# jamornsriwasansak/evplp

Hardware: AMD Instinct MI355X
Metric: Mpaths/s (higher is better)
Workload: dtype f32

## Files before the change

### evplp_amd/csrc/kernels.h

```cpp
#pragma once
#include "evplp_types.h"

namespace evplp {

struct PrimaryArgs {
    SceneDev sc; StripDev st; CamBasis cam;
    float jitter[2]; int32_t clear_light; int32_t pad;
    float4 *g_pos, *g_nrm, *g_dif, *g_phg, *g_light;
    float4 *tile_box;
    const char *cuts; int32_t cut_gw_log2, cut_gh_log2, cut_groups_x, pad2;
};
struct PrimaryCutArgs {
    const BvhNode *nodes; StripDev st; CamBasis cam;
    int32_t tiles_x, tiles_y, gw_log2, gh_log2, groups_x, groups_y;
    char *cuts;
};
void launch_primary_cuts(const PrimaryCutArgs &a, hipStream_t s);
#ifndef EVPLP_PRIMARY_BLOCKS
#define EVPLP_PRIMARY_BLOCKS 1
#endif
#ifndef EVPLP_PRIMARY_BLOCK_LOG2
#define EVPLP_PRIMARY_BLOCK_LOG2 2
#endif

struct LightTraceArgs {
    SceneDev sc;
    uint32_t rng_seed, path_begin, path_count, photons_per_path;
    evplp_record *records;
    int32_t *stack_overflow;
    uint32_t overflow_stride, pad;
};
#ifndef EVPLP_LT_STACK
#define EVPLP_LT_STACK 20
#endif
constexpr int kLtLdsStack = EVPLP_LT_STACK;
inline int lt_overflow_entries(const SceneDev &sc) {
    const int generic = 3 * ((sc.bvh_depth + 1) / 2) + 4;
    const int worst = sc.stack4_entries > 0 && sc.stack4_entries < generic ? sc.stack4_entries : generic;
    return worst > kLtLdsStack ? worst - kLtLdsStack : 0;
}

struct PassCounters {
    unsigned long long rays;
    unsigned long long nodes;
    unsigned long long pairs;
    unsigned long long aux;
    unsigned long long hist[64];
    unsigned long long shard_rays[64], shard_shaded[64];
    unsigned long long nonfinite;
};
#ifndef EVPLP_DEBUG_NAN
#define EVPLP_DEBUG_NAN 0
#endif
constexpr int kCounterShards = 64;

struct GatherArgs {
    SceneDev sc; StripDev st;
    const float4 *g_pos, *g_nrm, *g_dif, *g_phg;
    const evplp_record *vpls;
    const uint32_t *vpl_src_index;
    const uint32_t *nvpl;
    evplp_frame_params fp;
    float pdf_mc2; int32_t pad0;
    float4 *out;
    float4 *partial;
    size_t partial_stride;
    PassCounters *counters;
    int32_t splits_per_wave;
    int32_t block_h_log2;
    int32_t group_first, group_count;
    unsigned long long *vsl_masks; int32_t masks_per_split; int32_t pad1;
    const char *cuts; uint32_t cut_vpl_stride; int32_t cut_gw_log2, cut_gh_log2, cut_groups_x;
    int32_t band_first, band_rows, cut_group_row_first;
    int32_t item_deal;
    unsigned long long *block_cost;
};
struct AdaptArgs { const int4 *tiles; const float4 *snap; int32_t n1, pad; };
constexpr int kCutEntries = 8;
constexpr int kCutNodes = kCutEntries / 2;
constexpr int kCutSlotBytes = kCutNodes * 64;
struct CutArgs {
    const BvhNode *nodes;
    const float4 *tile_box;
    int32_t tiles_x, tiles_y;
    int32_t gw_log2, gh_log2;
    int32_t groups_x, groups_y;
    int32_t group_row_first, pad;
    const evplp_record *vpls; const uint32_t *nvpl; uint32_t vpl_stride;
    char *cuts;
    const int4 *adapt_tiles;
};
void launch_gather_cuts(const CutArgs &a, hipStream_t s);
void launch_tile_boxes(const StripDev &st, const float4 *g_pos, float4 *tile_box, int tiles_x, int tiles_y, hipStream_t s);
#ifndef EVPLP_VPL_SPLIT
#define EVPLP_VPL_SPLIT 128
#endif
constexpr int kVplSplit = EVPLP_VPL_SPLIT;
#ifndef EVPLP_GATHER_K
#define EVPLP_GATHER_K 2
#endif
constexpr int kDefaultSplitsPerWave = EVPLP_GATHER_K;

struct PathTraceArgs {
    SceneDev sc; StripDev st;
    const float4 *g_pos, *g_nrm, *g_dif, *g_phg;
    float camera_pos[3]; uint32_t rng_seed;
    uint32_t max_bounces, do_accumulate;
    float4 *out;
    PassCounters *counters;
};

constexpr int kPtBatchMaxSamples = 64;
constexpr int kPtBatchMaxTiles = 1 << 25;
constexpr size_t kPtBatchSlotBytes = 4 * 64 * sizeof(float4);
struct PtBatchSamples { float jitter[kPtBatchMaxSamples][2]; uint32_t seed[kPtBatchMaxSamples]; };
__host__ __device__ inline int32_t pt_tile_samples(int32_t mode, int4 r, int32_t S) {
    return mode == 0 ? S : mode == 1 ? (r.x == 0 ? S : 0) : (r.w < 0 || r.w > S ? S : r.w);
}
__host__ __device__ inline bool gather_tile_takes(int4 r, int32_t phase, int32_t S) {
    return r.w < 0 || phase < (r.w < S ? r.w : S);
}
constexpr int kGatherBudgetMaxWindow = 64;
void launch_gather_budget_mask(const int4 *tiles, int32_t ntiles, int32_t phase, int32_t window, int4 *mask, hipStream_t s);
void launch_gather_budget_step(int4 *tiles, const int4 *mask, int32_t ntiles, hipStream_t s);
void launch_gather_reduce_budget(const GatherArgs &a, int stencil_test, const int4 *tiles, const int4 *mask, float4 *snap, int32_t n1, hipStream_t s);
struct PtBatchChunk {
    const uint32_t *table; const int32_t *total;
    int32_t item_first, item_count;
    float4 *staging;
    unsigned long long cut_mask;
};
void launch_pt_batch_table(const int4 *tiles, int32_t ntiles, int32_t mode, int32_t samples, int32_t *first, uint32_t *table, hipStream_t s);
void launch_pt_batch_primary(const PrimaryArgs &a, const PtBatchSamples &sm, const PtBatchChunk &ch, hipStream_t s);
void launch_pt_batch_trace(const PathTraceArgs &a, const PtBatchSamples &sm, const PtBatchChunk &ch, hipStream_t s);
void launch_pt_batch_accumulate(const StripDev &st, float4 *plane, const int32_t *first, int32_t ntiles, const PtBatchChunk &ch, hipStream_t s);
void launch_pt_batch_close(const StripDev &st, int4 *tiles, int32_t mode, const int32_t *first, const float4 *snap, float4 *out, int32_t n_after, int32_t ntiles, hipStream_t s);

constexpr int kSummaryShards = 1024, kSummaryStride = 32, kSummaryFinal = kSummaryShards * kSummaryStride;
constexpr int kSummaryHeavy = kSummaryFinal + 8;
#ifndef EVPLP_BIN_CHUNKS
#define EVPLP_BIN_CHUNKS 1
#endif
constexpr int kBinChunks = EVPLP_BIN_CHUNKS;
constexpr int kBinGroup = 256 * kBinChunks;
constexpr int kSegCap = 4 * kBinGroup;
#ifndef EVPLP_SCATTER_G
#define EVPLP_SCATTER_G 2
#endif
constexpr int kScatterG = EVPLP_SCATTER_G;
constexpr int kMaxBuckets = 1024;
constexpr int kBucketTilesLog2 = 7;
constexpr int kMaxBucketTilesLog2 = 9;
struct SplatArgs {
    StripDev st; CamBasis cam;
    evplp_frame_params fp;
    const float4 *g_pos, *g_nrm, *g_dif, *g_phg;
    const evplp_record *records; uint32_t num_records;
    float4 *out;
    uint32_t *tile_pairs;
    float4 *tile_box;
    uint32_t *tile_cursor;
    uint32_t *bin_items;
    uint32_t bin_stride;
    uint32_t *seg;
    uint16_t *seg_off;
    uint32_t *big_list;
    uint32_t *big_count;
    int32_t num_bin_groups, bucket_w_log2, bucket_h_log2, buckets_x, num_buckets;
    uint32_t *bin_items_tmp;
    float4 *compact;
    uint32_t *overflow;
    uint32_t *summary;
    int32_t tiles_x, tiles_y; int32_t deterministic; int32_t boxes_valid;
    PassCounters *counters;
    const float4 *proxy_slabs; const float *proxy_hm; int32_t proxy_count; float proxy_rin, proxy_rout;
    uint32_t *tile_frags;
    uint32_t *heavy_list; uint8_t *tile_flags; uint32_t heavy_cap, heavy_threshold;
};
constexpr int kMaxProxySlabs = EVPLP_MAX_PROXY_PLANES;
constexpr float kProxyOpen = 1.0e15f;
constexpr int kSplatTile = 8;
constexpr int kCompactF4 = 4;

inline size_t lane_stack_bytes(const SceneDev &sc) { return (size_t)(sc.bvh_depth + 2) * 64 * sizeof(int32_t); }
inline size_t lane_stack_bytes4(const SceneDev &sc) {
    const int generic = 3 * ((sc.bvh_depth + 1) / 2) + 4;
    const int entries = sc.stack4_entries > 0 ? (sc.stack4_entries < generic ? sc.stack4_entries : generic) : generic;
    return (size_t)entries * 64 * sizeof(int32_t);
}

void launch_primary(const PrimaryArgs &a, hipStream_t s);
void launch_light_trace(const LightTraceArgs &a, hipStream_t s);
void launch_compact_vpl(const evplp_record *records, uint32_t nrec, evplp_record *out, uint32_t *src_index,
                        uint32_t *count_out, hipStream_t s);
void launch_gather_vpl_items(const GatherArgs &a, hipStream_t s, const AdaptArgs &ad = AdaptArgs{});
void launch_gather_vsl(const GatherArgs &a, hipStream_t s, const AdaptArgs &ad = AdaptArgs{});
int gather_launch_tiles(const GatherArgs &a);
void launch_gather_reduce(const GatherArgs &a, int stencil_test, hipStream_t s, const AdaptArgs &ad = AdaptArgs{});
void launch_gather_lvc(const GatherArgs &a, const evplp_record *records, hipStream_t s);
void launch_path_trace(const PathTraceArgs &a, hipStream_t s, const AdaptArgs &ad = AdaptArgs{});
void launch_splat_bin(const SplatArgs &a, hipStream_t s);
void launch_splat_tiles(const SplatArgs &a, bool split_tiles, hipStream_t s, hipEvent_t dominant_begin, hipEvent_t dominant_end);
void launch_resolve(const StripDev &st, const float4 *vpl, const float4 *pm, const float4 *light,
                    float vs, float ps, float ls, int mask_emitter, int gamma, float *out_rgb, hipStream_t s);
void launch_assemble_strips(const StripDev &st, int nranks, const uint32_t *owner, int chunk_rows, const float *gathered, float *frame, hipStream_t s, int channels = 3);
struct ShardPlanes { const float4 *p[64]; };
void launch_reduce_shards(const ShardPlanes &src, int n, int first_nonzero, size_t count, float4 *out, int num_cus, hipStream_t s);
void launch_fill_zero(void *p, size_t bytes, hipStream_t s);
struct RowError { double num, rel, rel_kept, kept; };
static_assert(sizeof(RowError) == 32, "RowError must be 32 bytes");
void launch_frame_error(const StripDev &st, const float *rgb, const float *ref, const uint8_t *keep, RowError *rows, hipStream_t s);
struct NoisePlanes { double *q; float4 *prev, *start; size_t stride; };
struct NoiseMoments { const double *q, *s; const float4 *prev, *start; size_t stride; };
void launch_noise_pool(const NoiseMoments &src, bool first, double *q, double *s_out, size_t n, hipStream_t s);
struct AdaptTiles { const int4 *tiles; int32_t tiles_x, pad; double n, scale; };
void launch_noise_fold(const NoisePlanes &m, const float4 *vpl, const float4 *pm, const StripDev &st, const AdaptTiles &at, int32_t k, hipStream_t s);
void launch_noise_rows(const StripDev &st, const NoiseMoments &m, double K, double B, double s2K, const float4 *light, float ls, int mask_emitter,
                       const float *rgb, const uint8_t *keep, RowError *rows, const AdaptTiles &at, hipStream_t s);
void launch_noise_variance(const StripDev &st, const NoiseMoments &m, double K, double B, double s2K, float *out_rgb, const AdaptTiles &at, hipStream_t s);
void launch_adaptive_retire(const StripDev &st, const NoiseMoments &m, double K, double B, double s2K, const float4 *light, float ls, int mask_emitter,
                            const float *rgb, double tau, int4 *tiles, int32_t tiles_x, int32_t tiles_y, int32_t n, const float4 *vpl, float4 *snap, hipStream_t s);

void launch_noise_fold_budget(const NoisePlanes &m, const StripDev &st, int4 *tiles, const float4 *snap, int32_t ntiles, hipStream_t s);
void launch_tile_noise(const StripDev &st, const NoiseMoments &m, double K, double B, double s2K, const float4 *light, float ls, int mask_emitter,
                       const float *rgb, const AdaptTiles &at, int32_t ntiles, double *out, hipStream_t s);

struct DenoisePixel { float4 u, pos, nrm, albedo, rgb; };
static_assert(sizeof(DenoisePixel) == 80, "DenoisePixel must be 80 bytes");
constexpr int kDenoiseFloats = (int)(sizeof(DenoisePixel) / sizeof(float));
void launch_denoise_prepare(const StripDev &st, const float *rgb, const float *var, const float4 *pos, const float4 *nrm, const float4 *dif,
                            const float4 *phg, const float4 *light, float4 *out, hipStream_t s);
struct DenoiseLevelArgs {
    const DenoisePixel *frame; const float4 *in; float4 *out;
    int32_t W, rows, in_step, h;
    float sigma_l, sigma_n, sigma_x_r, pad;
};
void launch_denoise_level(const DenoiseLevelArgs &a, hipStream_t s);
void launch_denoise_finish(const DenoisePixel *frame, const float4 *u, size_t n, float *out_rgb, hipStream_t s);

struct TemporalPrev { float4 pos, nrm; };
constexpr int kTemporalPrevFloats = (int)(sizeof(TemporalPrev) / sizeof(float));
void launch_prev_pose(const PrimaryArgs &a, const float *prev_v, TemporalPrev *prev, float4 *debug, hipStream_t s);
void launch_pose_snapshot(const TriAttr *attrs, int32_t ntri, float *prev_v, hipStream_t s);
int temporal_count_slots(int W, int rows);
struct TemporalArgs {
    DenoisePixel *frame; const TemporalPrev *prev; const float4 *h_in; float4 *h_out; uint4 *counts;
    size_t px;
    int32_t W, rows, H, has_history;
    CamBasis cam, prev_cam;
    float sigma_x_r, normal_cos, max_history, pad;
};
void launch_temporal_accumulate(const TemporalArgs &a, hipStream_t s);

}
// ... 1 lines not shown
```

### evplp_amd/csrc/kernels_gather.hip

```cpp
#include "device_common.hpp"
#include "kernels.h"
#include <algorithm>

namespace evplp {

constexpr int kRecF4 = sizeof(evplp_record) / 16;

struct Pixel {
    V3 p1, n1, rd, rs; float e; V3 wi10;
};

struct Vpl {
    V3 pos, n, flux, fdir, rd, rs; float psel, e;
};
EV_DEV Vpl load_vpl(const float4 *r) {
    Vpl v; float4 a = r[0], b = r[1], c = r[2], d = r[3], e = r[4], f = r[5];
    v.pos = v3(a); v.n = v3(b); v.psel = b.w; v.flux = v3(c); v.fdir = v3(d); v.rd = v3(e); v.rs = v3(f); v.e = f.w;
    return v;
}

EV_DEV float phong_eval_f_hw(V3 out, V3 in, V3 n, float e) {
    V3 r = reflect(-in, n);
    float d = fmaxf(dot(out, r), 0.0f);
    if (d <= 0.000001f) return 0.0f;
    return (e + 2.0f) * __builtin_amdgcn_exp2f(e * __builtin_amdgcn_logf(d)) * EV_INV_PI * 0.5f;
}

template <bool PXL = false>
EV_DEV V3 vpl_shade(const evplp_frame_params &fp, float pdf_mc2, const Pixel &px, const Vpl &v, V3 v12, float c1c2, const float *wi10_lds = nullptr, bool px_glossy = true) {
    float dist2 = dot(v12, v12);
    V3 wi12 = v12 * __builtin_amdgcn_rsqf(dist2);
    float ph2 = 0.0f;
    if (v.rs.x != 0.0f || v.rs.y != 0.0f || v.rs.z != 0.0f) {
        if (v.e == 0.0f) { V3 r = reflect(-v.fdir, v.n); ph2 = fmaxf(dot(-wi12, r), 0.0f) <= 0.000001f ? 0.0f : (v.e + 2.0f) * 1.0f * EV_INV_PI * 0.5f; }
        else ph2 = phong_eval_f_hw(-wi12, v.fdir, v.n, v.e);
    }
    float ph1 = 0.0f;
    V3 prs = PXL ? v3(0.f, 0.f, 0.f) : px.rs;
    if (PXL ? px_glossy : ballot64(px.rs.x != 0.0f || px.rs.y != 0.0f || px.rs.z != 0.0f) != 0ull) {
        ph1 = phong_eval_f_hw(wi10_lds ? v3(wi10_lds[0], wi10_lds[64], wi10_lds[128]) : px.wi10, wi12, px.n1, PXL ? wi10_lds[576] : px.e);
        if (PXL) prs = v3(wi10_lds[384], wi10_lds[448], wi10_lds[512]);
    }
    const V3 prd = PXL ? v3(wi10_lds[192], wi10_lds[256], wi10_lds[320]) : px.rd;
    V3 brdf2 = v.rd * EV_INV_PI + v.rs * ph2;
    V3 brdf1 = prd * EV_INV_PI + prs * ph1;
    float g21 = c1c2 * __builtin_amdgcn_rcpf(dist2 * dist2);
    const uint32_t mode = fp.mis_mode;
    if (mode == 0u) return v.flux * brdf1 * brdf2 * g21;
    if (mode <= 3u) {
        float pdf_de = g21 * EV_INV_PI * v.psel;
        if (!(v.rs.x <= 0.000001f))
            pdf_de += ph2 * ((v.e + 1.0f) * __builtin_amdgcn_rcpf(v.e + 2.0f)) * fmaxf(dot(px.n1, wi12), 0.0f) * __builtin_amdgcn_rcpf(dist2) * (1.0f - v.psel);
        float w;
        if (mode == 1u) w = fp.pdf_mc * __builtin_amdgcn_rcpf(fp.pdf_mc + pdf_de);
        else if (mode == 2u) w = fp.pdf_mc > pdf_de ? 1.0f : 0.0f;
        else { float a2 = pdf_mc2, b2 = pdf_de * pdf_de; w = a2 * __builtin_amdgcn_rcpf(a2 + b2); }
        return (v.flux * w) * brdf1 * brdf2 * g21;
    }
    if (mode == 4u) return (v.flux * fminf(g21, fp.clamping_value)) * brdf1 * brdf2;
    V3 x = (brdf1 * g21) * brdf2;
    x = v3(fminf(x.x, fp.clamping_value), fminf(x.y, fp.clamping_value), fminf(x.z, fp.clamping_value));
    return v.flux * x;
}

struct Item { int x, ly, gy, group; bool in_image, has_tile; uint32_t p; };
#ifndef EVPLP_GROUP_ORDER
#define EVPLP_GROUP_ORDER 0
#endif
#ifndef EVPLP_XCD_TIMES
#define EVPLP_XCD_TIMES 0
#endif
#ifndef EVPLP_XCD_ROTATE
#define EVPLP_XCD_ROTATE 2
#endif
struct ItemIx { int tx, ty, sg, tile_l, blk; };
template <bool RANGE = false>
EV_DEV ItemIx item_index(const GatherArgs &a, int b) {
    const int tiles_x = (a.st.W + 7) >> 3;
    const int groups = RANGE ? a.group_count : kVplSplit / a.splits_per_wave;
    const bool grp = EVPLP_GROUP_ORDER == 1 && a.cuts != nullptr;
    const int gwl = grp ? a.cut_gw_log2 : 0, ghl = grp ? a.cut_gh_log2 : 0, gl = gwl + ghl;
    const int xcd = b & 7, j = b >> 3;
    const int q = j & ((1 << gl) - 1);
    const int r = a.item_deal ? b : j >> gl;
    const int unit_j = r / groups;
    const int unit = a.item_deal ? unit_j : unit_j * 8 + xcd;
    const int shl = a.block_h_log2, bwl = 3 - gwl, bhl = shl - ghl, nbx = (tiles_x + 7) >> 3;
    const int l = unit & ((1 << (bwl + bhl)) - 1);
    ItemIx ix;
    ix.blk = a.band_first * nbx + (unit >> (bwl + bhl));
    const int rot = EVPLP_XCD_ROTATE == 0 ? 0 : EVPLP_XCD_ROTATE == 1 ? (l >> bwl) + ix.blk : (l >> bwl) + (ix.blk % nbx) + ((ix.blk / nbx) << bhl);
    const int ux = ((ix.blk % nbx) << bwl) | ((l + rot) & ((1 << bwl) - 1)), uy = ((ix.blk / nbx) << bhl) | (l >> bwl);
    ix.tx = (ux << gwl) | (q & ((1 << gwl) - 1)); ix.ty = (uy << ghl) | (q >> gwl);
    ix.sg = r - unit_j * groups;
    ix.tile_l = (unit << gl) | q;
    return ix;
}
template <bool RANGE = false>
EV_DEV Item item_setup(const GatherArgs &a, int lane, int b) {
    const StripDev &st = a.st;
    const int tiles_x = (st.W + 7) >> 3, tiles_y = (st.local_rows + 7) >> 3;
    const int sh = 1 << a.block_h_log2, nbx = (tiles_x + 7) >> 3, nby = (tiles_y + sh - 1) >> a.block_h_log2;
    const ItemIx ix = item_index<RANGE>(a, b);
    Item t;
    t.group = (RANGE ? a.group_first : 0) + ix.sg;
    t.has_tile = ix.blk < nbx * (a.band_rows > 0 ? min(nby, a.band_first + a.band_rows) : nby) && ix.tx < tiles_x && ix.ty < tiles_y;
    t.x = ix.tx * 8 + (lane & 7); t.ly = ix.ty * 8 + (lane >> 3);
    const int cly = max(min(t.ly, st.local_rows - 1), 0);
    t.gy = st.global_row(cly);
    t.has_tile = t.has_tile && __builtin_amdgcn_readfirstlane(t.gy) < st.H;
    t.in_image = t.has_tile && t.x < st.W && t.ly < st.local_rows && t.gy < st.H;
    t.p = (uint32_t)cly * (uint32_t)st.W + (uint32_t)min(t.x, st.W - 1);
    return t;
}

template <bool RANGE = false>
EV_DEV uint32_t item_texel(const GatherArgs &a, int lane, int b) {
    const StripDev &st = a.st;
    const ItemIx ix = item_index<RANGE>(a, b);
    const int x = ix.tx * 8 + (lane & 7), ly = ix.ty * 8 + (lane >> 3);
    return (uint32_t)max(min(ly, st.local_rows - 1), 0) * (uint32_t)st.W + (uint32_t)min(x, st.W - 1);
}

EV_DEV uint32_t item_cut_group(const GatherArgs &a, const Item &t) {
    const int tx = __builtin_amdgcn_readfirstlane(t.x) >> 3, ty = __builtin_amdgcn_readfirstlane(t.ly) >> 3;
    return (uint32_t)(((ty >> a.cut_gh_log2) - a.cut_group_row_first) * a.cut_groups_x + (tx >> a.cut_gw_log2));
}
EV_DEV bool tile_retired(const GatherArgs &a, const AdaptArgs &ad, const Item &t) {
    const int tx = __builtin_amdgcn_readfirstlane(t.x) >> 3, ty = __builtin_amdgcn_readfirstlane(t.ly) >> 3;
    const uint32_t off = (uint32_t)(ty * ((a.st.W + 7) >> 3) + tx) * (uint32_t)sizeof(int4);
    int nt;
    asm volatile("s_load_dword %0, %1, %2\n\ts_waitcnt lgkmcnt(0)" : "=s"(nt) : "s"(ad.tiles), "s"(off) : "memory");
    return nt != 0;
}

#ifndef EVPLP_CUT_RING
#define EVPLP_CUT_RING 3
#endif
#ifndef EVPLP_PX_LDS
#define EVPLP_PX_LDS 1
#endif
constexpr int kGatherPxFloats = 64 * (EVPLP_PX_LDS ? 10 : 3);
#ifndef EVPLP_GATHER_WAVES
#define EVPLP_GATHER_WAVES 8
#endif

EV_DEV Vpl fetch_vpl(const evplp_record *r) {
    const v16i ra = *reinterpret_cast<const v16i *>(r);
    const v8i rb = *reinterpret_cast<const v8i *>(reinterpret_cast<const int *>(r) + 16);
    Vpl v;
    v.pos = v3(f_of(ra[0]), f_of(ra[1]), f_of(ra[2])); v.n = v3(f_of(ra[4]), f_of(ra[5]), f_of(ra[6])); v.psel = f_of(ra[7]);
    v.flux = v3(f_of(ra[8]), f_of(ra[9]), f_of(ra[10])); v.fdir = v3(f_of(ra[12]), f_of(ra[13]), f_of(ra[14]));
    v.rd = v3(f_of(rb[0]), f_of(rb[1]), f_of(rb[2])); v.rs = v3(f_of(rb[4]), f_of(rb[5]), f_of(rb[6])); v.e = f_of(rb[7]);
    return v;
}
EV_DEV void fetch_vpl_head(const evplp_record *vpls, uint32_t i, V3 &pos, V3 &n, float &psel) {
    const v8i ra = sload8(vpls, i * (uint32_t)sizeof(evplp_record));
    pos = v3(f_of(ra[0]), f_of(ra[1]), f_of(ra[2])); n = v3(f_of(ra[4]), f_of(ra[5]), f_of(ra[6])); psel = f_of(ra[7]);
}
EV_DEV void fetch_vpl_tail(const evplp_record *vpls, uint32_t i, Vpl &v) {
    const v16i rb = sload16(vpls, i * (uint32_t)sizeof(evplp_record) + 32u);
    v.flux = v3(f_of(rb[0]), f_of(rb[1]), f_of(rb[2])); v.fdir = v3(f_of(rb[4]), f_of(rb[5]), f_of(rb[6]));
    v.rd = v3(f_of(rb[8]), f_of(rb[9]), f_of(rb[10])); v.rs = v3(f_of(rb[12]), f_of(rb[13]), f_of(rb[14])); v.e = f_of(rb[15]);
}

#if EVPLP_GATHER_TIMES
__device__ unsigned long long g_gather_times[2 * 131072];
extern "C" int evplp_debug_gather_times(unsigned long long *out, int n) { return (int)hipMemcpyFromSymbol(out, HIP_SYMBOL(g_gather_times), sizeof(unsigned long long) * (size_t)n); }
#endif
EV_DEV void item_cost_add(const GatherArgs &a, int ty, unsigned long long t0, int waves) {
    const unsigned long long dt = __builtin_amdgcn_s_memrealtime() - t0;
    if (threadIdx.x == 0) atomicAdd(&a.block_cost[(ty * 8) / a.st.strip_rows], dt * 8ull / (unsigned long long)waves);
}
template <bool CUT, bool COST = false, bool ADAPT = false>
__attribute__((amdgpu_num_vgpr(kWalkKernelVgprs)))
__global__ __launch_bounds__(64, EVPLP_GATHER_WAVES) void gather_vpl_kernel(GatherArgs a, AdaptArgs ad) {
    unsigned long long t_cost = 0ull;
    if constexpr (COST) t_cost = __builtin_amdgcn_s_memrealtime();
#if EVPLP_GATHER_TIMES
    const unsigned long long t_start = __builtin_amdgcn_s_memrealtime();
#endif
    extern __shared__ float s_dyn[];
    float *const s_wi10 = s_dyn, *const s_lvl = s_dyn + kGatherPxFloats;
    const int lane = threadIdx.x;
    const Item t = item_setup(a, lane, (int)blockIdx.x);
    if (!t.has_tile) return;
    if constexpr (ADAPT) { if (tile_retired(a, ad, t)) return; }
    const uint32_t p = t.p;

    Pixel px;
    float4 gp = a.g_pos[p], gn = a.g_nrm[p], gd = a.g_dif[p], gs = a.g_phg[p];
    px.p1 = v3(gp); px.n1 = v3(gn); px.rd = v3(gd); px.rs = v3(gs); px.e = gs.w;
#ifndef EVPLP_WI10_LDS
#define EVPLP_WI10_LDS 1
#endif
    {
        const V3 w = normalize(v3(a.fp.camera_pos) - px.p1);
        s_wi10[lane] = w.x; s_wi10[64 + lane] = w.y; s_wi10[128 + lane] = w.z;
        px.wi10 = EVPLP_WI10_LDS ? v3(0.f, 0.f, 0.f) : w;
    }
    bool px_glossy = true;
    if constexpr (EVPLP_PX_LDS != 0) {
        static_assert(EVPLP_WI10_LDS != 0, "EVPLP_PX_LDS continues the LDS column of the view direction");
        s_wi10[192 + lane] = px.rd.x; s_wi10[256 + lane] = px.rd.y; s_wi10[320 + lane] = px.rd.z;
        s_wi10[384 + lane] = px.rs.x; s_wi10[448 + lane] = px.rs.y; s_wi10[512 + lane] = px.rs.z; s_wi10[576 + lane] = px.e;
        px_glossy = ballot64(px.rs.x != 0.0f || px.rs.y != 0.0f || px.rs.z != 0.0f) != 0ull;
        px.rd = v3(0.f, 0.f, 0.f); px.rs = v3(0.f, 0.f, 0.f); px.e = 0.0f;
    }
    const bool valid = t.in_image && gp.w != 0.0f;

    const uint32_t nvpl = *a.nvpl;
    const int k = a.splits_per_wave;
    const char *node_base = pinned(reinterpret_cast<const char *>(a.sc.nodes)), *leaf_base = pinned(reinterpret_cast<const char *>(a.sc.leaves));
    const evplp_record *vpls = pinned(a.vpls);
    const char *cuts_g = nullptr;
    if constexpr (CUT) cuts_g = pinned(a.cuts + (size_t)item_cut_group(a, t) * a.cut_vpl_stride * (size_t)kCutSlotBytes);
    V3 total = v3(0.f, 0.f, 0.f);
    uint32_t rays = t.in_image ? 0x80000000u : 0u, shaded = 0;
#if EVPLP_TRAVERSAL_STATS
    int32_t cache_leaf = kNoChild; bool prev_all_occ = false;
#endif
    constexpr bool kRing = CUT && kWalkAsm;
    constexpr int kRingSlots = EVPLP_CUT_RING, kAhead = kRingSlots - 1;
    __shared__ float4 s_cut[kRing ? kRingSlots : 1][kCutSlotBytes / 16];
    int pj = 0; uint32_t pi = (uint32_t)(t.group * k), qslot = 0u;
    auto ring_skip_empty = [&]() { while (pj < k && pi >= nvpl) { pj++; pi = (uint32_t)(t.group * k + pj); } };
    auto ring_issue = [&](uint32_t slot) {
        if (lane < kCutSlotBytes / 16) lds_dma16(cuts_g + (size_t)pi * kCutSlotBytes + (size_t)lane * 16u, lds_offset(&s_cut[slot][0]));
        pi += (uint32_t)kVplSplit; ring_skip_empty();
    };
    if constexpr (kRing) {
        ring_skip_empty();
        for (int q = 0; q < kAhead; q++) if (pj < k) ring_issue((uint32_t)q);
    }
    for (int jj = 0; jj < k; jj++) {
        const uint32_t split = (uint32_t)(t.group * k + jj);
        V3 result = v3(0.f, 0.f, 0.f);
        for (uint32_t i = split; i < nvpl; i += kVplSplit) {
            const float4 *cut_lds = nullptr;
            if constexpr (kRing) {
                if (pj < k) { ring_issue((qslot + (uint32_t)kAhead) % (uint32_t)kRingSlots); wait_vmcnt<kAhead>(); }
                else wait_vmcnt0();
                cut_lds = &s_cut[qslot][0];
                qslot = (qslot + 1u) % (uint32_t)kRingSlots;
            }
            V3 vpos, vn; float vpsel; fetch_vpl_head(vpls, i, vpos, vn, vpsel);
            V3 v12 = vpos - px.p1;
            float c1 = fmaxf(dot_exact(px.n1, v12), 0.0f);
            float c2 = fmaxf(-dot_exact(vn, v12), 0.0f);
            float c1c2 = c1 * c2;
            bool active = valid && !(c1c2 <= 0.0f);
            if (ballot64(active) == 0ull) continue;
            rays += active ? 1u : 0u;
            bool occ;
            {
#if EVPLP_TRAVERSAL_STATS
                unsigned long long cache_kill = 0ull;
                const unsigned long long act_m = ballot64(active);
                if (cache_leaf != kNoChild) {
                    const LeafOps L = fetch_leaf(leaf_base, (uint32_t)cache_leaf);
                    const V3 dd = -v12;
                    bool any = tri_pair_any(L.A, vpos, dd, 0.0001f, 1.0f - 0.0001f);
                    if (L.cnt > 2u) any = any | tri_pair_any(L.B, vpos, dd, 0.0001f, 1.0f - 0.0001f);
                    cache_kill = ballot64(any) & act_m;
                }
                WalkStats ws = { 0u, 0u, 0u, 0u, kNoChild, 0u };
                occ = occluded_wave_ref<CUT, true>(node_base, leaf_base, vpos, -v12, 0.0001f, 1.0f - 0.0001f, active, &ws, cuts_g, i * (uint32_t)kCutSlotBytes);
                const bool all_occ = ballot64(active && !occ) == 0ull;
                const unsigned long long occ_m = ballot64(active && occ);
                if (lane == 0) {
                    atomicAdd(&a.counters->hist[41], (unsigned long long)__builtin_popcountll(occ_m));
                    atomicAdd(&a.counters->nodes, (unsigned long long)ws.nodes);
                    atomicAdd(&a.counters->aux, (unsigned long long)ws.syn);
                    atomicAdd(&a.counters->hist[min(ws.leaves, 31u)], 1ull);
                    atomicAdd(&a.counters->hist[32], 1ull);
                    atomicAdd(&a.counters->hist[33], (unsigned long long)ws.pairs);
                    if (all_occ) { atomicAdd(&a.counters->hist[34], 1ull); atomicAdd(&a.counters->hist[36], (unsigned long long)ws.nodes); atomicAdd(&a.counters->hist[37], (unsigned long long)ws.leaves); }
                    if (ws.leaves == 0u) atomicAdd(&a.counters->hist[35], (unsigned long long)ws.nodes);
                    if (cache_leaf != kNoChild) {
                        atomicAdd(&a.counters->hist[42], 1ull);
                        atomicAdd(&a.counters->hist[40], (unsigned long long)__builtin_popcountll(cache_kill));
                        if (cache_kill == act_m) { atomicAdd(&a.counters->hist[38], 1ull); atomicAdd(&a.counters->hist[39], (unsigned long long)ws.nodes); }
                        if (prev_all_occ) { atomicAdd(&a.counters->hist[44], 1ull); if (cache_kill == act_m) atomicAdd(&a.counters->hist[43], 1ull); }
                    }
                    atomicAdd(&a.counters->hist[45 + min(ws.nodes / 16u, 18u)], 1ull);
                }
                if (ws.hit_leaf != kNoChild) cache_leaf = ws.hit_leaf;
                prev_all_occ = all_occ;
#else
                if constexpr (kWalkAsm) occ = occluded_wave<CUT>(node_base, leaf_base, vpos, -v12, 0.0001f, 1.0f - 0.0001f, active, cut_lds, i * (uint32_t)kCutSlotBytes);
                else occ = occluded_wave_ref<CUT>(node_base, leaf_base, vpos, -v12, 0.0001f, 1.0f - 0.0001f, active, nullptr, cuts_g, i * (uint32_t)kCutSlotBytes);
#endif
            }
            const bool lit = active && !occ;
            if (ballot64(lit) == 0ull) continue;
            Vpl v; fetch_vpl_head(vpls, i, v.pos, v.n, v.psel); fetch_vpl_tail(vpls, i, v);
            evplp_frame_params fps; float pdf_mc2;
            {
                const void *ka = (const void *)__builtin_amdgcn_kernarg_segment_ptr();
                typedef int v4i_ __attribute__((ext_vector_type(4)));
                v4i_ q; int q2;
                asm volatile("s_load_dwordx4 %0, %2, %3\n\ts_load_dword %1, %2, %4\n\ts_waitcnt lgkmcnt(0)" : "=&s"(q), "=&s"(q2)
                             : "s"(ka), "s"((uint32_t)(offsetof(GatherArgs, fp) + offsetof(evplp_frame_params, mis_mode))), "s"((uint32_t)offsetof(GatherArgs, pdf_mc2)) : "memory");
                fps.mis_mode = (uint32_t)q[0]; fps.pdf_mc = f_of(q[1]); fps.clamping_value = f_of(q[2]); pdf_mc2 = f_of(q2);
            }
            if (lit) { result = result + vpl_shade<EVPLP_PX_LDS != 0>(fps, pdf_mc2, px, v, v12, c1c2, EVPLP_WI10_LDS ? s_wi10 + lane : nullptr, px_glossy); shaded++; }
        }
        {
            int lev = 0;
            while ((jj >> lev) & 1) {
                float *q = s_lvl + lev * 192 + lane;
                result = v3(q[0], q[64], q[128]) + result;
                lev++;
            }
            float *q = s_lvl + lev * 192 + lane;
            q[0] = result.x; q[64] = result.y; q[128] = result.z;
        }
        total = result;
    }
#if EVPLP_DEBUG_NAN
    if ((rays >> 31) != 0u && !(isfinite(total.x) && isfinite(total.y) && isfinite(total.z))) atomicAdd(&a.counters->nonfinite, 1ull);
#endif
#if EVPLP_XCD_TIMES
    if (lane == 0) atomicMax(&a.counters->hist[16 + (blockIdx.x & 7u)], (unsigned long long)__builtin_amdgcn_s_memrealtime());
#endif
#if EVPLP_GATHER_TIMES
    if (lane == 0 && (blockIdx.x & 15u) == 0u && (blockIdx.x >> 4) < 131072u) { g_gather_times[2 * (blockIdx.x >> 4)] = t_start; g_gather_times[2 * (blockIdx.x >> 4) + 1] = __builtin_amdgcn_s_memrealtime(); }
#endif
    int lane_out = lane, blk_out = (int)blockIdx.x;
    asm volatile("" : "+v"(lane_out), "+s"(blk_out));
    const bool in_image = (rays >> 31) != 0u;
    rays &= 0xffffu;
    if (in_image) a.partial[(size_t)item_index(a, blk_out).sg * a.partial_stride + item_texel(a, lane_out, blk_out)] = make_float4(total.x, total.y, total.z, __uint_as_float(rays | (shaded << 16)));
    if constexpr (COST) item_cost_add(a, item_index(a, blk_out).ty, t_cost, EVPLP_GATHER_WAVES);
}

EV_DEV float4 reduce_out(V3 r, float inv, float acc, float4 old) {
    return make_float4(r.x / inv + acc * old.x, r.y / inv + acc * old.y, r.z / inv + acc * old.z, 0.0f + acc * old.w);
}
EV_DEV int pixel_tile(const StripDev &st, int ly, size_t i) { return (ly >> 3) * ((st.W + 7) >> 3) + ((int)(i - (size_t)ly * st.W) >> 3); }
EV_DEV V3 reduce_tree(const GatherArgs &a, size_t i, unsigned long long &rays, unsigned long long &shaded) {
    const int groups = kVplSplit / a.splits_per_wave;
    V3 r = v3(0.f, 0.f, 0.f), lv0 = r, lv1 = r, lv2 = r, lv3 = r, lv4 = r, lv5 = r, lv6 = r;
    for (int g = 0; g < groups; g++) {
        float4 q = a.partial[(size_t)g * a.partial_stride + i];
        const uint32_t st = __float_as_uint(q.w);
        rays += st & 0xffffu; shaded += st >> 16;
        r = v3(q.x, q.y, q.z);
#define EV_MERGE(L, NEXT) if (((g >> L) & 1) == 0) lv##L = r; else { r = lv##L + r; NEXT }
        EV_MERGE(0, EV_MERGE(1, EV_MERGE(2, EV_MERGE(3, EV_MERGE(4, EV_MERGE(5, EV_MERGE(6, ;)))))))
#undef EV_MERGE
    }
    return r;
}
EV_DEV void reduce_counters(const GatherArgs &a, unsigned long long rays, unsigned long long shaded) {
    __shared__ unsigned long long s_sum[2];
    if (threadIdx.x < 2) s_sum[threadIdx.x] = 0ull;
    __syncthreads();
    for (int off = 32; off > 0; off >>= 1) { rays += __shfl_down(rays, off); shaded += __shfl_down(shaded, off); }
    if ((threadIdx.x & 63) == 0) { atomicAdd(&s_sum[0], rays); atomicAdd(&s_sum[1], shaded); }
    __syncthreads();
    if (threadIdx.x == 0) {
        const int shard = blockIdx.x & (kCounterShards - 1);
        atomicAdd(&a.counters->shard_rays[shard], s_sum[0]);
        atomicAdd(&a.counters->shard_shaded[shard], s_sum[1]);
    }
}
template <bool ADAPT = false>
__global__ __launch_bounds__(256) void gather_reduce_kernel(GatherArgs a, int stencil_test, AdaptArgs ad) {
    const size_t i = (size_t)blockIdx.x * 256 + threadIdx.x;
    const size_t n = (size_t)a.st.W * a.st.local_rows;
    unsigned long long rays = 0ull, shaded = 0ull;
    bool writes = i < n;
    int nt = 0;
    if (writes) {
        const int ly = (int)(i / a.st.W);
        if (a.st.global_row(ly) >= a.st.H) writes = false;
        else {
            if constexpr (ADAPT) nt = ad.tiles[pixel_tile(a.st, ly, i)].x;
            if (nt == 0 && stencil_test && a.g_pos[i].w == 0.0f) writes = false;
        }
    }
    if (ADAPT && writes && nt != 0) {
        a.out[i] = extrapolate(ad.snap[i], ad.n1, nt);
    } else if (writes) {
        const V3 r = reduce_tree(a, i, rays, shaded);
        a.out[i] = reduce_out(r, (float)a.fp.num_vpl_light_paths, (float)a.fp.do_accumulate, a.out[i]);
    }
    reduce_counters(a, rays, shaded);
}

__global__ __launch_bounds__(256) void gather_budget_mask_kernel(const int4 *tiles, int32_t ntiles, int32_t phase, int32_t window, int4 *mask) {
    const int t = (int)(blockIdx.x * 256 + threadIdx.x);
    if (t >= ntiles) return;
    const int4 r = tiles[t];
    const bool takes = gather_tile_takes(r, phase, window);
    mask[t] = make_int4(takes ? 0 : max(r.x, 1), takes ? 1 : 0, 0, 0);
}
__global__ __launch_bounds__(256) void gather_budget_step_kernel(int4 *tiles, const int4 *mask, int32_t ntiles) {
    const int t = (int)(blockIdx.x * 256 + threadIdx.x);
    if (t >= ntiles) return;
    if (mask[t].y != 0) tiles[t].x += 1;
}
__global__ __launch_bounds__(256) void gather_reduce_budget_kernel(GatherArgs a, int stencil_test, const int4 *tiles, const int4 *mask, float4 *snap, int32_t n1) {
    const size_t i = (size_t)blockIdx.x * 256 + threadIdx.x;
    const size_t n = (size_t)a.st.W * a.st.local_rows;
    unsigned long long rays = 0ull, shaded = 0ull;
    bool in_image = i < n, sums = false;
    int nt = 0;
    if (in_image) {
        const int ly = (int)(i / a.st.W);
        if (a.st.global_row(ly) >= a.st.H) in_image = false;
        else {
            const int t = pixel_tile(a.st, ly, i);
            const bool takes = mask[t].y != 0;
            nt = tiles[t].x + (takes ? 1 : 0);
            sums = takes && !(stencil_test && a.g_pos[i].w == 0.0f);
        }
    }
    if (in_image) {
        float4 R = snap[i];
        if (sums) {
            const V3 r = reduce_tree(a, i, rays, shaded);
            R = reduce_out(r, (float)a.fp.num_vpl_light_paths, (float)a.fp.do_accumulate, R);
            snap[i] = R;
        }
        a.out[i] = nt > 0 ? extrapolate(R, n1, nt) : R;
    }
    reduce_counters(a, rays, shaded);
}

#ifndef EVPLP_LVC_WIDE
#define EVPLP_LVC_WIDE 0
#endif
#if EVPLP_LVC_WIDE
#define LVC_OCCLUDED occluded_lane4
#else
#define LVC_OCCLUDED occluded_lane
#endif
#ifndef EVPLP_LVC_SPEC
#define EVPLP_LVC_SPEC 0
#endif
#ifndef EVPLP_LVC_WAVES
#define EVPLP_LVC_WAVES 6
#endif
__global__ __launch_bounds__(64, EVPLP_LVC_WAVES) void gather_lvc_kernel(GatherArgs a, const evplp_record *records) {
    extern __shared__ int32_t lds_stack[];
    __shared__ unsigned long long s_stats[2];
    const int lane = threadIdx.x;
    if (lane < 2) s_stats[lane] = 0ull;
    const int tiles_x = (a.st.W + 7) >> 3;
    const int tx = blockIdx.x % tiles_x, ty = blockIdx.x / tiles_x;
    const int x = tx * 8 + (lane & 7);
    const int ly = ty * 8 + (lane >> 3);
    if (x >= a.st.W || ly >= a.st.local_rows) return;
    const int y = a.st.global_row(ly);
    if (y >= a.st.H) return;
    const size_t p = (size_t)ly * a.st.W + x;
    Pixel px;
    float4 gp = a.g_pos[p], gn = a.g_nrm[p], gd = a.g_dif[p], gs = a.g_phg[p];
    if (gp.w == 0.0f) return;
    px.p1 = v3(gp); px.n1 = v3(gn); px.rd = v3(gd); px.rs = v3(gs); px.e = gs.w;
    px.wi10 = normalize(v3(a.fp.camera_pos) - px.p1);
    int32_t *stack = lds_stack + lane;

    Rng rng; rng_init(rng, (uint32_t)y * (uint32_t)a.st.W + (uint32_t)x, a.fp.rng_seed, 0x4c564300u);
#ifndef EVPLP_LVC_NO_OFFSET
#define EVPLP_LVC_NO_OFFSET 0
#endif
// ... 280 lines not shown
__global__ __launch_bounds__(64, EVPLP_VSL_WAVES) void gather_vsl_shade_kernel(GatherArgs a, AdaptArgs ad) {
    unsigned long long t_cost = 0ull;
    if constexpr (COST) t_cost = __builtin_amdgcn_s_memrealtime();
    extern __shared__ float s_lvl[];
    __shared__ unsigned long long s_lit[kVslChunk];
    const int lane = threadIdx.x;
    const int W = a.st.W;
    const Item t = item_setup<true>(a, lane, (int)blockIdx.x);
    if (!t.has_tile) return;
    if constexpr (ADAPT) { if (tile_retired(a, ad, t)) return; }
    const bool valid = t.in_image;
    const uint32_t pixel_id = (uint32_t)t.gy * (uint32_t)W + (uint32_t)t.x;
    const uint64_t pixel_key = vsl_key(((uint64_t)a.fp.rng_seed << 32) | (uint64_t)pixel_id);
    const uint32_t nvpl = *a.nvpl;
    const int k = a.splits_per_wave;
    const evplp_record *vpls = pinned(a.vpls);
    const int tile_l = launch_tile(a);
    const unsigned long long *masks = a.vsl_masks + vsl_mask_base(a, tile_l, t.group);
    Pixel px;
    { const float4 gp = a.g_pos[t.p], gn = a.g_nrm[t.p], gd = a.g_dif[t.p], gs = a.g_phg[t.p]; px.p1 = v3(gp); px.n1 = v3(gn); px.rd = v3(gd); px.rs = v3(gs); px.e = gs.w; }
    px.wi10 = normalize(v3(a.fp.camera_pos) - px.p1);
    VslPixel P;
    {
        const float ml = max_color(px.rd), mp = max_color(px.rs);
        P.dead = ml + mp <= 0.000001f; P.psel = ml / (mp + ml);
        P.glossy = px.rs.x != 0.0f || px.rs.y != 0.0f || px.rs.z != 0.0f; P.pdf_glossy = !(px.rs.x <= 0.000001f);
        P.R1 = reflect(-px.wi10, px.n1);
    }
    V3 total = v3(0.f, 0.f, 0.f);
    uint32_t cnt = 0;
    for (int jj = 0; jj < k; jj++) {
        const uint32_t split = (uint32_t)(t.group * k + jj);
        V3 result = v3(0.f, 0.f, 0.f);
        uint32_t cbase = 0;
        for (uint32_t first = split; first < nvpl; first += (uint32_t)(kVplSplit * kVslChunk), cbase += (uint32_t)kVslChunk) {
            const uint32_t n = min((uint32_t)kVslChunk, (nvpl - first + (uint32_t)kVplSplit - 1u) / (uint32_t)kVplSplit);
            uint32_t moff = (uint32_t)jj * (uint32_t)a.masks_per_split + cbase;
            asm volatile("" : "+s"(moff));
            const unsigned long long *src = masks + moff;
            uint32_t q0 = (uint32_t)lane;
            asm volatile("" : "+v"(q0));
            for (uint32_t q = q0; q < n; q += 64u) s_lit[q] = src[q];
            for (uint32_t c = 0; c < n; c++) {
                const unsigned long long lit = s_lit[c];
                const uint32_t lo = __builtin_amdgcn_readfirstlane((uint32_t)lit), hi = __builtin_amdgcn_readfirstlane((uint32_t)(lit >> 32));
                if ((lo | hi) == 0u) continue;
                const uint32_t i = first + c * (uint32_t)kVplSplit;
                Vpl v; fetch_vpl_head(vpls, i, v.pos, v.n, v.psel); fetch_vpl_tail(vpls, i, v);
                const bool lit_lane = (((lane < 32 ? lo : hi) >> (lane & 31)) & 1u) != 0u;
                const uint64_t record_key = vsl_key((uint64_t)(1u + a.vpl_src_index[i]) * 0xD1B54A32D192ED03ull);
                const bool diffuse_wave = !(v.rs.x != 0.0f || v.rs.y != 0.0f || v.rs.z != 0.0f) && ballot64(lit_lane && (P.glossy || P.psel < 1.0f)) == 0ull;
                if (lit_lane) {
                    const V3 v12 = v.pos - px.p1;
                    const float inv_dist = vslm::rsq(dot(v12, v12));
                    const V3 nv12 = v12 * inv_dist;
                    VslCtx cx;
                    const float rdratio = a.fp.vsl_radius * inv_dist;
                    cx.half_cone = (rdratio >= 1.0f) ? EV_PI / 2.0f : asinf(rdratio);
                    cx.cos_half_cone = (rdratio >= 1.0f) ? cosf(EV_PI / 2.0f) : vslm::fsqrt(1.0f - rdratio * rdratio);
                    cx.solid_angle = EV_PI * 2.0f * (1.0f - cx.cos_half_cone);
                    cx.inv_solid_angle = vslm::rcp(cx.solid_angle);
                    cx.inv_pi_r2 = a.fp.vsl_inv_pi_radius2; cx.nd12 = nv12;
                    const int num_samples = (int)(cx.half_cone / EV_PI * 2.0f * 100.0f) + 1;
                    cnt += ((uint32_t)num_samples << 12) + 1u;
                    VslRng rng = vsl_rng_seed(pixel_key, record_key);
                    VslLight L;
                    {
                        const float ml = max_color(v.rd), mp = max_color(v.rs);
                        L.dead = ml + mp <= 0.000001f; L.psel = ml * vslm::rcp(mp + ml);
                        L.glossy = v.rs.x != 0.0f || v.rs.y != 0.0f || v.rs.z != 0.0f; L.pdf_glossy = !(v.rs.x <= 0.000001f);
                        L.R2 = reflect(-v.fdir, v.n);
                    }
                    VslFrames F;
                    F.nd_n1 = onb_local(vslm::fonb_make(px.n1), nv12); F.nd_r1 = onb_local(vslm::fonb_make(P.R1), nv12);
                    F.nd_n2 = onb_local(vslm::fonb_make(v.n), -nv12);  F.nd_r2 = onb_local(vslm::fonb_make(L.R2), -nv12);
                    const Onb cone = vslm::fonb_make(nv12);
                    V3 acc = v3(0.f, 0.f, 0.f);
                    if (diffuse_wave) {
                        float acc_d = 0.0f;
                        for (int sidx = 0; sidx < num_samples; sidx++) {
                            vsl_sample_cone<true>(px, v, P, L, cx, cone, acc, acc_d, rng);
                            vsl_sample_brdf1<true>(px, v, P, L, cx, F, acc, rng);
                            vsl_sample_brdf2<true>(px, v, P, L, cx, F, acc, rng);
                        }
                        acc = acc + ((px.rd * EV_INV_PI) * (v.rd * EV_INV_PI)) * acc_d;
                    } else {
                        float unused = 0.0f;
                        for (int sidx = 0; sidx < num_samples; sidx++) {
                            vsl_sample_cone<false>(px, v, P, L, cx, cone, acc, unused, rng);
                            vsl_sample_brdf1<false>(px, v, P, L, cx, F, acc, rng);
                            vsl_sample_brdf2<false>(px, v, P, L, cx, F, acc, rng);
                        }
                    }
                    acc = (v.flux * cx.inv_pi_r2) * acc;
                    result = result + acc * vslm::rcp((float)num_samples);
                }
            }
        }
        {
            int lev = 0;
            while ((jj >> lev) & 1) {
                float *q = s_lvl + lev * 192 + lane;
                result = v3(q[0], q[64], q[128]) + result;
                lev++;
            }
            float *q = s_lvl + lev * 192 + lane;
            q[0] = result.x; q[64] = result.y; q[128] = result.z;
        }
        total = result;
    }
#if EVPLP_DEBUG_NAN
    if (valid && !(isfinite(total.x) && isfinite(total.y) && isfinite(total.z))) atomicAdd(&a.counters->nonfinite, 1ull);
#endif
#if EVPLP_XCD_TIMES
    if (lane == 0) atomicMax(&a.counters->hist[16 + (blockIdx.x & 7u)], (unsigned long long)__builtin_amdgcn_s_memrealtime());
#endif
    const uint32_t nlit = cnt & 4095u;
    uint32_t nsamp = cnt >> 12;
    for (int off = 32; off > 0; off >>= 1) nsamp += __shfl_down(nsamp, off);
    if (lane == 0) atomicAdd(&a.counters->hist[blockIdx.x & 63u], (unsigned long long)nsamp);
    int lane_out = lane, blk_out = (int)blockIdx.x;
    asm volatile("" : "+v"(lane_out), "+s"(blk_out));
    const int group_out = a.group_first + item_index<true>(a, blk_out).sg;
    if (valid) a.partial[(size_t)group_out * a.partial_stride + item_texel<true>(a, lane_out, blk_out)] = make_float4(total.x, total.y, total.z, __uint_as_float(nlit << 16));
    if constexpr (COST) item_cost_add(a, item_index<true>(a, blk_out).ty, t_cost, EVPLP_VSL_WAVES);
}

int gather_launch_tiles(const GatherArgs &a) {
    const int tiles_x = (a.st.W + 7) / 8, tiles_y = (a.st.local_rows + 7) / 8, sh = 1 << a.block_h_log2;
    const int nby = (tiles_y + sh - 1) / sh, rows = a.band_rows > 0 ? std::min(a.band_rows, nby - a.band_first) : nby;
    return ((tiles_x + 7) / 8) * std::max(rows, 0) * 8 * sh;
}
static dim3 gather_grid(const GatherArgs &a) {
    const int groups = a.group_count > 0 ? a.group_count : kVplSplit / a.splits_per_wave;
    return dim3((unsigned)(gather_launch_tiles(a) * groups));
}
void launch_gather_reduce(const GatherArgs &a, int stencil_test, hipStream_t s, const AdaptArgs &ad) {
    size_t n = (size_t)a.st.W * a.st.local_rows;
    if (ad.tiles) hipLaunchKernelGGL(gather_reduce_kernel<true>, dim3((unsigned)((n + 255) / 256)), dim3(256), 0, s, a, stencil_test, ad);
    else hipLaunchKernelGGL(gather_reduce_kernel<false>, dim3((unsigned)((n + 255) / 256)), dim3(256), 0, s, a, stencil_test, ad);
}
void launch_gather_budget_mask(const int4 *tiles, int32_t ntiles, int32_t phase, int32_t window, int4 *mask, hipStream_t s) {
    if (ntiles <= 0) return;
    hipLaunchKernelGGL(gather_budget_mask_kernel, dim3((unsigned)((ntiles + 255) / 256)), dim3(256), 0, s, tiles, ntiles, phase, window, mask);
}
void launch_gather_budget_step(int4 *tiles, const int4 *mask, int32_t ntiles, hipStream_t s) {
    if (ntiles <= 0) return;
    hipLaunchKernelGGL(gather_budget_step_kernel, dim3((unsigned)((ntiles + 255) / 256)), dim3(256), 0, s, tiles, mask, ntiles);
}
void launch_gather_reduce_budget(const GatherArgs &a, int stencil_test, const int4 *tiles, const int4 *mask, float4 *snap, int32_t n1, hipStream_t s) {
    const size_t n = (size_t)a.st.W * a.st.local_rows;
    hipLaunchKernelGGL(gather_reduce_budget_kernel, dim3((unsigned)((n + 255) / 256)), dim3(256), 0, s, a, stencil_test, tiles, mask, snap, n1);
}
static size_t fold_lds_bytes(const GatherArgs &a, int extra_floats) {
    int levels = 1; while ((1 << (levels - 1)) < a.splits_per_wave) levels++;
    return (size_t)(levels * 192 + extra_floats) * sizeof(float);
}
void launch_gather_vpl_items(const GatherArgs &a, hipStream_t s, const AdaptArgs &ad) {
    const size_t lds = fold_lds_bytes(a, kGatherPxFloats);
    if (ad.tiles && !a.block_cost) {
        if (a.cuts) hipLaunchKernelGGL((gather_vpl_kernel<true, false, true>), gather_grid(a), dim3(64), lds, s, a, ad);
        else hipLaunchKernelGGL((gather_vpl_kernel<false, false, true>), gather_grid(a), dim3(64), lds, s, a, ad);
        return;
    }
    if (a.block_cost) {
        if (a.cuts) hipLaunchKernelGGL((gather_vpl_kernel<true, true>), gather_grid(a), dim3(64), lds, s, a, ad);
        else hipLaunchKernelGGL((gather_vpl_kernel<false, true>), gather_grid(a), dim3(64), lds, s, a, ad);
    } else if (a.cuts) hipLaunchKernelGGL((gather_vpl_kernel<true>), gather_grid(a), dim3(64), lds, s, a, ad);
    else hipLaunchKernelGGL((gather_vpl_kernel<false>), gather_grid(a), dim3(64), lds, s, a, ad);
}
void launch_gather_vsl(const GatherArgs &a, hipStream_t s, const AdaptArgs &ad) {
    if (a.block_cost) {
        if (a.cuts) hipLaunchKernelGGL((gather_vsl_walk_kernel<true, true>), gather_grid(a), dim3(64), 0, s, a, ad);
        else hipLaunchKernelGGL((gather_vsl_walk_kernel<false, true>), gather_grid(a), dim3(64), 0, s, a, ad);
        hipLaunchKernelGGL((gather_vsl_shade_kernel<true>), gather_grid(a), dim3(64), fold_lds_bytes(a, 0), s, a, ad);
        return;
    }
    if (ad.tiles) {
        if (a.cuts) hipLaunchKernelGGL((gather_vsl_walk_kernel<true, false, true>), gather_grid(a), dim3(64), 0, s, a, ad);
        else hipLaunchKernelGGL((gather_vsl_walk_kernel<false, false, true>), gather_grid(a), dim3(64), 0, s, a, ad);
        hipLaunchKernelGGL((gather_vsl_shade_kernel<false, true>), gather_grid(a), dim3(64), fold_lds_bytes(a, 0), s, a, ad);
        return;
    }
    if (a.cuts) hipLaunchKernelGGL((gather_vsl_walk_kernel<true>), gather_grid(a), dim3(64), 0, s, a, ad);
    else hipLaunchKernelGGL((gather_vsl_walk_kernel<false>), gather_grid(a), dim3(64), 0, s, a, ad);
    hipLaunchKernelGGL((gather_vsl_shade_kernel<false>), gather_grid(a), dim3(64), fold_lds_bytes(a, 0), s, a, ad);
}

}
```

Before: 46960.

## Stream VPL records into LDS ring alongside cut slots via shared DMA

```diff
diff --git a/evplp_amd/csrc/kernels.h b/evplp_amd/csrc/kernels.h
--- a/evplp_amd/csrc/kernels.h
+++ b/evplp_amd/csrc/kernels.h
@@ -100,6 +100,16 @@
 #define EVPLP_GATHER_K 2
 #endif
 constexpr int kDefaultSplitsPerWave = EVPLP_GATHER_K;
+#ifndef EVPLP_PX_LDS
+#define EVPLP_PX_LDS 1
+#endif
+constexpr int kGatherPxFloats = 64 * (EVPLP_PX_LDS ? 10 : 3);
+constexpr size_t gather_fold_lds_bytes(int k, int px_floats, bool top_level) {
+    int levels = 1;
+    while ((1 << (levels - 1)) < k) levels++;
+    return (size_t)((top_level ? levels : levels - 1) * 192 + px_floats) * sizeof(float);
+}
+constexpr size_t gather_vpl_lds_bytes(int k) { return gather_fold_lds_bytes(k, kGatherPxFloats, false); }
 
 struct PathTraceArgs {
     SceneDev sc; StripDev st;
diff --git a/evplp_amd/csrc/kernels_gather.hip b/evplp_amd/csrc/kernels_gather.hip
--- a/evplp_amd/csrc/kernels_gather.hip
+++ b/evplp_amd/csrc/kernels_gather.hip
@@ -137,10 +137,12 @@
 #ifndef EVPLP_CUT_RING
 #define EVPLP_CUT_RING 3
 #endif
-#ifndef EVPLP_PX_LDS
-#define EVPLP_PX_LDS 1
-#endif
-constexpr int kGatherPxFloats = 64 * (EVPLP_PX_LDS ? 10 : 3);
+#ifndef EVPLP_VPL_RING
+#define EVPLP_VPL_RING 1
+#endif
+#ifndef EVPLP_TAIL_PROBE
+#define EVPLP_TAIL_PROBE 0
+#endif
 #ifndef EVPLP_GATHER_WAVES
 #define EVPLP_GATHER_WAVES 8
 #endif
@@ -158,6 +160,14 @@
     const v8i ra = sload8(vpls, i * (uint32_t)sizeof(evplp_record));
     pos = v3(f_of(ra[0]), f_of(ra[1]), f_of(ra[2])); n = v3(f_of(ra[4]), f_of(ra[5]), f_of(ra[6])); psel = f_of(ra[7]);
 }
+#if EVPLP_TAIL_PROBE
+EV_DEV void fetch_vpl_head_probe(const evplp_record *vpls, uint32_t i, V3 &pos, V3 &n, float &psel) {
+    v8i ra; int warm;
+    asm volatile("s_load_dwordx8 %0, %2, %3\n\ts_load_dword %1, %2, %3 offset:0x20\n\ts_load_dword %1, %2, %3 offset:0x40\n\ts_waitcnt lgkmcnt(0)"
+                 : "=&s"(ra), "=&s"(warm) : "s"(vpls), "s"(i * (uint32_t)sizeof(evplp_record)));
+    pos = v3(f_of(ra[0]), f_of(ra[1]), f_of(ra[2])); n = v3(f_of(ra[4]), f_of(ra[5]), f_of(ra[6])); psel = f_of(ra[7]);
+}
+#endif
 EV_DEV void fetch_vpl_tail(const evplp_record *vpls, uint32_t i, Vpl &v) {
     const v16i rb = sload16(vpls, i * (uint32_t)sizeof(evplp_record) + 32u);
     v.flux = v3(f_of(rb[0]), f_of(rb[1]), f_of(rb[2])); v.fdir = v3(f_of(rb[4]), f_of(rb[5]), f_of(rb[6]));
@@ -221,12 +231,20 @@
     int32_t cache_leaf = kNoChild; bool prev_all_occ = false;
 #endif
     constexpr bool kRing = CUT && kWalkAsm;
+    constexpr bool kRecRing = kRing && EVPLP_VPL_RING != 0;
     constexpr int kRingSlots = EVPLP_CUT_RING, kAhead = kRingSlots - 1;
-    __shared__ float4 s_cut[kRing ? kRingSlots : 1][kCutSlotBytes / 16];
+    constexpr int kSlotF4 = kCutSlotBytes / 16, kRingF4 = kSlotF4 + (kRecRing ? kRecF4 : 0);
+    static_assert(kSlotF4 == 16 && kRecF4 == 6 && kRingF4 <= 64, "one DMA instruction moves slot and record: 16 + 6 lanes of 16 bytes");
+    __shared__ float4 s_cut[kRing ? kRingSlots : 1][kRingF4];
     int pj = 0; uint32_t pi = (uint32_t)(t.group * k), qslot = 0u;
     auto ring_skip_empty = [&]() { while (pj < k && pi >= nvpl) { pj++; pi = (uint32_t)(t.group * k + pj); } };
+    const uintptr_t ring_lane_base = lane < kSlotF4 ? (uintptr_t)cuts_g + (uintptr_t)lane * 16u : (uintptr_t)vpls + (uintptr_t)(lane - kSlotF4) * 16u;
+    const uint32_t ring_lane_stride = lane < kSlotF4 ? (uint32_t)kCutSlotBytes : (uint32_t)sizeof(evplp_record);
     auto ring_issue = [&](uint32_t slot) {
-        if (lane < kCutSlotBytes / 16) lds_dma16(cuts_g + (size_t)pi * kCutSlotBytes + (size_t)lane * 16u, lds_offset(&s_cut[slot][0]));
+        if constexpr (kRecRing) {
+            const uintptr_t src = ring_lane_base + (uintptr_t)pi * (uintptr_t)ring_lane_stride;
+            if (lane < kRingF4) lds_dma16(reinterpret_cast<const void *>(src), lds_offset(&s_cut[slot][0]));
+        } else if (lane < kSlotF4) lds_dma16(cuts_g + (size_t)pi * kCutSlotBytes + (size_t)lane * 16u, lds_offset(&s_cut[slot][0]));
         pi += (uint32_t)kVplSplit; ring_skip_empty();
     };
     if constexpr (kRing) {
@@ -244,7 +262,12 @@
                 cut_lds = &s_cut[qslot][0];
                 qslot = (qslot + 1u) % (uint32_t)kRingSlots;
             }
-            V3 vpos, vn; float vpsel; fetch_vpl_head(vpls, i, vpos, vn, vpsel);
+            V3 vpos, vn; float vpsel;
+            if constexpr (kRecRing) { const float4 h0 = cut_lds[kSlotF4], h1 = cut_lds[kSlotF4 + 1]; vpos = v3(h0); vn = v3(h1); vpsel = h1.w; }
+#if EVPLP_TAIL_PROBE
+            else if constexpr (kRing) fetch_vpl_head_probe(vpls, i, vpos, vn, vpsel);
+#endif
+            else fetch_vpl_head(vpls, i, vpos, vn, vpsel);
             V3 v12 = vpos - px.p1;
             float c1 = fmaxf(dot_exact(px.n1, v12), 0.0f);
             float c2 = fmaxf(-dot_exact(vn, v12), 0.0f);
@@ -294,16 +317,31 @@
             }
             const bool lit = active && !occ;
             if (ballot64(lit) == 0ull) continue;
-            Vpl v; fetch_vpl_head(vpls, i, v.pos, v.n, v.psel); fetch_vpl_tail(vpls, i, v);
-            evplp_frame_params fps; float pdf_mc2;
-            {
-                const void *ka = (const void *)__builtin_amdgcn_kernarg_segment_ptr();
-                typedef int v4i_ __attribute__((ext_vector_type(4)));
-                v4i_ q; int q2;
-                asm volatile("s_load_dwordx4 %0, %2, %3\n\ts_load_dword %1, %2, %4\n\ts_waitcnt lgkmcnt(0)" : "=&s"(q), "=&s"(q2)
-                             : "s"(ka), "s"((uint32_t)(offsetof(GatherArgs, fp) + offsetof(evplp_frame_params, mis_mode))), "s"((uint32_t)offsetof(GatherArgs, pdf_mc2)) : "memory");
-                fps.mis_mode = (uint32_t)q[0]; fps.pdf_mc = f_of(q[1]); fps.clamping_value = f_of(q[2]); pdf_mc2 = f_of(q2);
+            Vpl v; evplp_frame_params fps; float pdf_mc2;
+            typedef int v4i_ __attribute__((ext_vector_type(4)));
+            const void *ka = (const void *)__builtin_amdgcn_kernarg_segment_ptr();
+            constexpr uint32_t kFpOff = (uint32_t)(offsetof(GatherArgs, fp) + offsetof(evplp_frame_params, mis_mode)), kMc2Off = (uint32_t)offsetof(GatherArgs, pdf_mc2);
+            v4i_ q; int q2;
+            if constexpr (kRecRing) {
+                typedef float v3f_ __attribute__((ext_vector_type(3)));
+                typedef float v4f_ __attribute__((ext_vector_type(4)));
+                v4f_ h1, t3; v3f_ t0, t1, t2;
+                asm volatile("s_load_dwordx4 %[q], %[ka], %[o1]\n\ts_load_dword %[q2], %[ka], %[o2]\n\t"
+                             "ds_read_b128 %[h1], %[ad] offset:%[c1]\n\tds_read_b96 %[t0], %[ad] offset:%[c2]\n\tds_read_b96 %[t1], %[ad] offset:%[c3]\n\t"
+                             "ds_read_b96 %[t2], %[ad] offset:%[c4]\n\tds_read_b128 %[t3], %[ad] offset:%[c5]\n\ts_waitcnt lgkmcnt(0)"
+                             : [q] "=&s"(q), [q2] "=&s"(q2), [h1] "=&v"(h1), [t0] "=&v"(t0), [t1] "=&v"(t1), [t2] "=&v"(t2), [t3] "=&v"(t3)
+                             : [ka] "s"(ka), [o1] "s"(kFpOff), [o2] "s"(kMc2Off), [ad] "v"(lds_offset(cut_lds)),
+                               [c1] "n"(kCutSlotBytes + 16), [c2] "n"(kCutSlotBytes + 32), [c3] "n"(kCutSlotBytes + 48), [c4] "n"(kCutSlotBytes + 64), [c5] "n"(kCutSlotBytes + 80)
+                             : "memory");
+                auto uni = [](float x) { return f_of(__builtin_amdgcn_readfirstlane(__float_as_int(x))); };
+                v.pos = vpos; v.n = v3(h1.x, h1.y, h1.z); v.psel = h1.w;
+                v.flux = v3(t0.x, t0.y, t0.z); v.fdir = v3(t1.x, t1.y, t1.z); v.rd = v3(t2.x, t2.y, t2.z);
+                v.rs = v3(uni(t3.x), uni(t3.y), uni(t3.z)); v.e = uni(t3.w);
+            } else {
+                fetch_vpl_head(vpls, i, v.pos, v.n, v.psel); fetch_vpl_tail(vpls, i, v);
+                asm volatile("s_load_dwordx4 %0, %2, %3\n\ts_load_dword %1, %2, %4\n\ts_waitcnt lgkmcnt(0)" : "=&s"(q), "=&s"(q2) : "s"(ka), "s"(kFpOff), "s"(kMc2Off) : "memory");
             }
+            fps.mis_mode = (uint32_t)q[0]; fps.pdf_mc = f_of(q[1]); fps.clamping_value = f_of(q[2]); pdf_mc2 = f_of(q2);
             if (lit) { result = result + vpl_shade<EVPLP_PX_LDS != 0>(fps, pdf_mc2, px, v, v12, c1c2, EVPLP_WI10_LDS ? s_wi10 + lane : nullptr, px_glossy); shaded++; }
         }
         {
@@ -313,8 +351,10 @@
                 result = v3(q[0], q[64], q[128]) + result;
                 lev++;
             }
-            float *q = s_lvl + lev * 192 + lane;
-            q[0] = result.x; q[64] = result.y; q[128] = result.z;
+            if (jj != k - 1) {
+                float *q = s_lvl + lev * 192 + lane;
+                q[0] = result.x; q[64] = result.y; q[128] = result.z;
+            }
         }
         total = result;
     }
@@ -901,12 +941,9 @@
     const size_t n = (size_t)a.st.W * a.st.local_rows;
     hipLaunchKernelGGL(gather_reduce_budget_kernel, dim3((unsigned)((n + 255) / 256)), dim3(256), 0, s, a, stencil_test, tiles, mask, snap, n1);
 }
-static size_t fold_lds_bytes(const GatherArgs &a, int extra_floats) {
-    int levels = 1; while ((1 << (levels - 1)) < a.splits_per_wave) levels++;
-    return (size_t)(levels * 192 + extra_floats) * sizeof(float);
-}
+static size_t fold_lds_bytes(const GatherArgs &a, int extra_floats) { return gather_fold_lds_bytes(a.splits_per_wave, extra_floats, true); }
 void launch_gather_vpl_items(const GatherArgs &a, hipStream_t s, const AdaptArgs &ad) {
-    const size_t lds = fold_lds_bytes(a, kGatherPxFloats);
+    const size_t lds = gather_vpl_lds_bytes(a.splits_per_wave);
     if (ad.tiles && !a.block_cost) {
         if (a.cuts) hipLaunchKernelGGL((gather_vpl_kernel<true, false, true>), gather_grid(a), dim3(64), lds, s, a, ad);
         else hipLaunchKernelGGL((gather_vpl_kernel<false, false, true>), gather_grid(a), dim3(64), lds, s, a, ad);
```

After: 48140 (median of 6 runs). +2.5%, better.
